# cgtuebingen/3D-RE-GEN

Measured on AMD Instinct MI355X. Metric: objects/sec (50-step Hunyuan3D-2 DiT + 256^3 marching cubes), higher is better.
Workload: dtype bf16; 1 GPU; configs[1]: 5 synthetic 512x512 RGBA crops per GPU, Hunyuan3D-2 full dims bf16, 50 flow-matching steps x CFG 2, 257^3 grid query + Lewiner marching cubes; weights=seeded synthetic, objects_total=5, objects_per_launch=4, parallelism=object-parallel x1

## Files before the change

### 3d-re-gen_amd/csrc/attn.hip

```cpp
#include <hip/hip_runtime.h>
#include <cstdio>
#include <stddef.h>
#include <stdint.h>

#include <type_traits>

#include "kernels.h"
#include "prof.h"

namespace r3g {
namespace {

typedef __attribute__((ext_vector_type(8))) __bf16 bf16x8;
typedef __attribute__((ext_vector_type(4))) __bf16 bf16x4;
typedef __attribute__((ext_vector_type(16))) float f32x16;
typedef __attribute__((ext_vector_type(8))) float f32x8;

constexpr int KV_TILE = 64;
constexpr int TILE_B = KV_TILE * 64 * 2;
constexpr int STAGE_B = 2 * TILE_B;

typedef __attribute__((ext_vector_type(2))) __bf16 bf16x2;
typedef __attribute__((ext_vector_type(2))) float f32x2;

__device__ __forceinline__ uint32_t pack_bf16(float a, float b) {
    const f32x2 v = {a, b};
    const bf16x2 h = __builtin_convertvector(v, bf16x2);
    return *reinterpret_cast<const uint32_t*>(&h);
}
// ... 42 lines not shown
                                                            offsetof(AttnEntry, lq));
}
__device__ __forceinline__ AttnEntry attn_entry(const AttnArgs& p, int e) {
    AttnEntry r{};
    if (!p.ragged) {
        r.lq = p.Lq; r.lk = p.Lk; r.bias_key = -1; r.buf = e;
        return r;
    }
    typedef const char __attribute__((address_space(4)))* kernarg_ptr;
    kernarg_ptr ka = (kernarg_ptr)__builtin_amdgcn_kernarg_segment_ptr();
    const AttnEntry __attribute__((address_space(4)))* t =
        (const AttnEntry __attribute__((address_space(4)))*)(ka + offsetof(AttnArgs, ent) + (size_t)e * sizeof(AttnEntry));
    r.lq = t->lq; r.lk = t->lk; r.bias_key = t->bias_key; r.bias_log2 = t->bias_log2; r.buf = t->buf;
    return r;
}
__device__ __forceinline__ int64_t attn_entry_out_row(int e, int q) {
    typedef const char __attribute__((address_space(4)))* kernarg_ptr;
    kernarg_ptr ka = (kernarg_ptr)__builtin_amdgcn_kernarg_segment_ptr();
    const AttnEntry __attribute__((address_space(4)))* t =
        (const AttnEntry __attribute__((address_space(4)))*)(ka + offsetof(AttnArgs, ent) + (size_t)e * sizeof(AttnEntry));
    const int split = t->o_split;
    return q < split ? t->o_row0 + q : t->o_row_split + (q - split);
}
template <int QT>
__device__ __forceinline__ void attn_work_item(const AttnArgs& p, int item, int& eb, int& hd, int& qt) {
    if (p.ragged) {
        int per_head = 0;
        for (int e = 0; e < p.B; ++e) per_head += (attn_entry_lq(p, e) + QT - 1) / QT;
        hd = item / per_head;
        int rem = item - hd * per_head;
        eb = 0;
        for (;;) {
            const int n = (attn_entry_lq(p, eb) + QT - 1) / QT;
            if (rem < n || eb + 1 >= p.B) break;
            rem -= n;
            ++eb;
        }
        qt = rem;
    } else {
        const int ntq0 = (p.Lq + QT - 1) / QT;
        const int per_head = ntq0 * p.B;
        hd = item / per_head;
        const int rem = item - hd * per_head;
        eb = rem / ntq0;
        qt = rem - eb * ntq0;
    }
}

template <bool GLDS, int ABL = 0>
__global__ __launch_bounds__(256, 2) void attn_kernel(AttnArgs p) {
    __shared__ __attribute__((aligned(16))) char smem[2 * STAGE_B];
    const int tid = threadIdx.x, lane = tid & 63;
    const int wid = __builtin_amdgcn_readfirstlane(tid >> 6);
    const int hd = blockIdx.y;
    const int eb = blockIdx.z;
    const AttnEntry en = attn_entry(p, eb);
    const int b = en.buf;
    const int ql = lane & 31, hh = lane >> 5;
    const int q = blockIdx.x * 128 + wid * 32 + ql;
    const int Lq = en.lq, Lk = en.lk;
    if ((int)blockIdx.x * 128 >= Lq) return;
    const int kvb = p.kv_batch_stride_zero ? 0 : b;
// ... 391 lines not shown
__device__ __forceinline__ float sum16(const float (&pe)[16]) {
    typedef __attribute__((ext_vector_type(2))) float f2;
    f2 ps = (f2){pe[0], pe[1]};
#pragma unroll
    for (int r = 2; r < 16; r += 2) ps += (f2){pe[r], pe[r + 1]};
    return ps[0] + ps[1];
}
constexpr float SCORE_LIMIT = 8.f;

__device__ __forceinline__ f32x16 mfma_32x32x16_fresh(const bf16x8& a, const bf16x8& b, const f32x16& c) {
    f32x16 d;
    asm volatile("s_nop 1\n\tv_mfma_f32_32x32x16_bf16 %0, %1, %2, %3" : "=&v"(d) : "v"(a), "v"(b), "v"(c));
    return d;
}

template <bool GLDS, bool PIPE, int NW, int ABL = 0, int VAR = 0>
__global__ __launch_bounds__(NW * 64, (PIPE || NW == 8) ? 2 : 3) void attn2_kernel(AttnArgs p) {
    __shared__ __attribute__((aligned(16))) char smem[(PIPE ? 3 : 2) * STAGE_B];
    const int tid = threadIdx.x, lane = tid & 63;
    const int wid = __builtin_amdgcn_readfirstlane(tid >> 6);
    const int ql = lane & 31, hh = lane >> 5;
    int eb, hd, qt;
    {
        const int nwg = gridDim.x, orig = blockIdx.x;
        const int qn = nwg >> 3, rn = nwg & 7, xcd = orig & 7;
        const int item = (xcd < rn ? xcd * (qn + 1) : rn * (qn + 1) + (xcd - rn) * qn) + (orig >> 3);
        constexpr int QT = NW * 32;
        attn_work_item<QT>(p, item, eb, hd, qt);
    }
    const AttnEntry en = attn_entry(p, eb);
    const int b = en.buf;
    const int q = qt * (NW * 32) + wid * 32 + ql;
    const int Lq = en.lq, Lk = en.lk;
    const int kvb = p.kv_batch_stride_zero ? 0 : b;
    const uint16_t* Qg = p.Q + (((int64_t)b * p.H + hd) * p.Lq_pad) * 64;
    const uint16_t* Kg = p.K + (((int64_t)kvb * p.H + hd) * p.Lk_pad) * 64;
    const uint16_t* Vtg = p.Vt + (((int64_t)kvb * p.H + hd) * 64) * (int64_t)p.Lk_pad;

    bf16x8 qf[4];
    {
        const int qrow = q < p.Lq_pad ? q : p.Lq_pad - 1;
#pragma unroll
        for (int ks = 0; ks < 4; ++ks)
            qf[ks] = *reinterpret_cast<const bf16x8*>(Qg + (int64_t)qrow * 64 + ks * 16 + hh * 8);
    }
    if (!p.q_prescaled) {
        const float sc = p.scale * 1.4426950408889634f;
#pragma unroll
        for (int ks = 0; ks < 4; ++ks) {
            union { bf16x8 v; uint32_t u[4]; } w;
            w.v = qf[ks];
// ... 32 lines not shown
    auto stage = [&](int t, char* dst) {
        if constexpr (GLDS) {
            const char* kt = reinterpret_cast<const char*>(Kg + (int64_t)t * (KV_TILE * 64));
            const char* vt = reinterpret_cast<const char*>(Vtg + (int64_t)t * KV_TILE);
#pragma unroll
            for (int i = 0; i < PPW; ++i) {
                if constexpr ((VAR & 4) != 0) {
                    lds_dma16_unseen(kt, koff[i], smem_lds + (uint32_t)(dst - smem) + (wid * PPW + i) * 1024);
                    lds_dma16_unseen(vt, voff[i], smem_lds + (uint32_t)(dst - smem) + TILE_B + (wid * PPW + i) * 1024);
                    continue;
                }
                __builtin_amdgcn_global_load_lds((const __attribute__((address_space(1))) void*)(kt + (size_t)koff[i]),
                                                 (__attribute__((address_space(3))) void*)(dst + (wid * PPW + i) * 1024), 16, 0, 0);
                __builtin_amdgcn_global_load_lds((const __attribute__((address_space(1))) void*)(vt + (size_t)voff[i]),
                                                 (__attribute__((address_space(3))) void*)(dst + TILE_B + (wid * PPW + i) * 1024),
                                                 16, 0, 0);
            }
        } else {
            static_assert(GLDS || NW == 4, "register staging is only built for 4-wave workgroups");
            stage_kv<false>(Kg, Vtg, p.Lk_pad, t * KV_TILE, dst, wid, lane, tid);
        }
    };
    const bool pad_tail = ntiles * KV_TILE > Lk;
    if constexpr (PIPE) {
        auto qk = [&](const char* buf, int kb, bool from_zero) {
            f32x16 sc_;
            const bf16x8 k0 = *reinterpret_cast<const bf16x8*>(buf + off[kb]);
            if (from_zero) {
                f32x16 z;
#pragma unroll
                for (int r = 0; r < 16; ++r) z[r] = 0.f;
                sc_ = __builtin_amdgcn_mfma_f32_32x32x16_bf16(k0, qf[0], z, 0, 0, 0);
            } else {
                sc_ = mfma_32x32x16_fresh(k0, qf[0], negm);
            }
#pragma unroll
            for (int ks = 1; ks < 4; ++ks) {
                const bf16x8 kf = *reinterpret_cast<const bf16x8*>(buf + (off[kb] ^ (ks << 5)));
                sc_ = __builtin_amdgcn_mfma_f32_32x32x16_bf16(kf, qf[ks], sc_, 0, 0, 0);
            }
            return sc_;
        };
        auto mask_block = [&](f32x16& sc_, int t, int kb) {
            const int key_base = t * KV_TILE + kb * 32 + 4 * hh;
#pragma unroll
            for (int r = 0; r < 16; ++r) {
// ... 72 lines not shown
                if (t > 0) mask_block(sA, t, 0);
                mask_block(sB, t, 1);
            }
            softmax_block(sA, &sB, pk);
            pv(cur, 0, pk);
            if constexpr (decltype(has_next)::value) {
                sA = qk(nxt, 0, false);
                softmax_block(sB, &sA, pk);
            } else {
                softmax_block(sB, nullptr, pk);
            }
            pv(cur, 1, pk);
            asm volatile("s_waitcnt vmcnt(0)" ::: "memory");
            __syncthreads();
        };
        int slot = 0;
        for (int t = 0; t < ntiles - 1; ++t) {
            tile(std::false_type{}, std::true_type{}, t, slot);
            slot = slot == 2 ? 0 : slot + 1;
        }
        if (pad_tail) tile(std::true_type{}, std::false_type{}, ntiles - 1, slot);
        else tile(std::false_type{}, std::false_type{}, ntiles - 1, slot);
    } else {
    unsigned long long sticky = 0;
    const unsigned long long valid_lanes = __ballot(q < Lq);
    auto pass = [&](auto FAST) __attribute__((always_inline)) {
    constexpr bool kFast = decltype(FAST)::value;
#pragma unroll
    for (int r = 0; r < 16; ++r) { o[0][r] = 0.f; o[1][r] = 0.f; negm[r] = 0.f; }
    m_run = 0.f;
    l_run = 0.f;
    stage(0, smem);
    asm volatile("s_waitcnt vmcnt(0)" ::: "memory");
    __syncthreads();

    auto tile = [&](auto masked, auto first, const int t) {
        const char* cur = smem + (t & 1) * STAGE_B;
        if constexpr ((VAR & 4) != 0) __builtin_amdgcn_s_waitcnt(0x0F70);
        if (!(ABL & 16) && t + 1 < ntiles) stage(t + 1, smem + ((t + 1) & 1) * STAGE_B);
#pragma unroll
        for (int kb = 0; kb < 2; ++kb) {
            constexpr bool kFirst = decltype(first)::value;
            const bool first_block = kFirst && kb == 0;
            f32x16 s;
            if constexpr ((ABL & 8) != 0) {
                const float tv = __int_as_float(0x3f800000 + (t << 8));
#pragma unroll
                for (int r = 0; r < 16; ++r) s[r] = negm[r] + tv * (float)(r + 1) * 1e-3f;
                if (!(ABL & 128)) {
#pragma unroll
                    for (int ks = 0; ks < 4; ++ks) {
                        const bf16x8 kf = *reinterpret_cast<const bf16x8*>(cur + (off[kb] ^ (ks << 5)));
                        asm volatile("" ::"v"(kf));
                    }
                }
            } else {
                const bf16x8 k0 = (ABL & 128) ? qf[1] : *reinterpret_cast<const bf16x8*>(cur + off[kb]);
                if (first_block) {
                    f32x16 z;
#pragma unroll
                    for (int r = 0; r < 16; ++r) z[r] = 0.f;
                    s = __builtin_amdgcn_mfma_f32_32x32x16_bf16(k0, qf[0], z, 0, 0, 0);
                } else {
                    s = mfma_32x32x16_fresh(k0, qf[0], negm);
                }
#pragma unroll
// ... 113 lines not shown
        pk[J - 1] = pack_bf16(st.ea, st.eb);
        asm volatile("" : "+v"(pk[J - 1]));
    }
    st.ea = a;
    st.eb = b;
    if (J == 7) {
        pk[7] = pack_bf16(a, b);
        st.ps0 += a;
        st.ps1 += b;
        asm volatile("" : "+v"(pk[7]));
    }
    asm volatile("" : "+v"(st.ps0), "+v"(st.ps1), "+v"(st.ea), "+v"(st.eb));
}

template <int NW, int VAR = 0>
__global__ __launch_bounds__(NW * 64, 2) void attn3_kernel(AttnArgs p) {
    __shared__ __attribute__((aligned(16))) char smem[2 * STAGE_B];
    const int tid = threadIdx.x, lane = tid & 63;
    const int wid = __builtin_amdgcn_readfirstlane(tid >> 6);
    const int ql = lane & 31, hh = lane >> 5;
    constexpr int QT = NW * 64;
    int eb, hd, qt;
    {
        const int nwg = gridDim.x, orig = blockIdx.x;
        const int qn = nwg >> 3, rn = nwg & 7, xcd = orig & 7;
        const int item = (xcd < rn ? xcd * (qn + 1) : rn * (qn + 1) + (xcd - rn) * qn) + (orig >> 3);
        attn_work_item<QT>(p, item, eb, hd, qt);
    }
    const AttnEntry en = attn_entry(p, eb);
    const int b = en.buf;
    const int q0 = qt * QT + wid * 64 + ql;
    const int Lq = en.lq, Lk = en.lk;
    const int kvb = p.kv_batch_stride_zero ? 0 : b;
    const uint16_t* Qg = p.Q + (((int64_t)b * p.H + hd) * p.Lq_pad) * 64;
    const uint16_t* Kg = p.K + (((int64_t)kvb * p.H + hd) * p.Lk_pad) * 64;
    const uint16_t* Vtg = p.Vt + (((int64_t)kvb * p.H + hd) * 64) * (int64_t)p.Lk_pad;

    bf16x8 qf[2][4];
#pragma unroll
    for (int qb = 0; qb < 2; ++qb) {
        const int q = q0 + qb * 32;
        const int qrow = q < p.Lq_pad ? q : p.Lq_pad - 1;
#pragma unroll
        for (int ks = 0; ks < 4; ++ks)
            qf[qb][ks] = *reinterpret_cast<const bf16x8*>(Qg + (int64_t)qrow * 64 + ks * 16 + hh * 8);
    }
    if (!p.q_prescaled) {
        const float sc = p.scale * 1.4426950408889634f;
#pragma unroll
        for (int qb = 0; qb < 2; ++qb)
// ... 251 lines not shown
                odd.y = pack_bf16(o[qb][db][8 * gp + 6] * inv, o[qb][db][8 * gp + 7] * inv);
                const u32x2 rx = __builtin_amdgcn_permlane32_swap(even.x, odd.x, false, false);
                const u32x2 ry = __builtin_amdgcn_permlane32_swap(even.y, odd.y, false, false);
                uint4 out;
                out.x = rx[0]; out.y = ry[0]; out.z = rx[1]; out.w = ry[1];
                if (q < Lq) *reinterpret_cast<uint4*>(dst + db * 32 + 16 * gp + 8 * hh) = out;
            }
    }
}


template <bool STAMP, int PRIO>
__global__ __launch_bounds__(768, 3) void attn6_kernel(AttnArgs p, unsigned long long* __restrict__ stamps) {
    extern __shared__ __attribute__((aligned(16))) char smem6[];
    char* const smem = smem6;
    constexpr int R = 4;
    const int tid = threadIdx.x, lane = tid & 63;
    const int wid = __builtin_amdgcn_readfirstlane(tid >> 6);
    const int grp = wid >> 2;
    const int ql = lane & 31, hh = lane >> 5;
    constexpr int QT = 384;
    int eb, hd, qt;
    {
        const int nwg = gridDim.x, orig = blockIdx.x;
        const int qn = nwg >> 3, rn = nwg & 7, xcd = orig & 7;
        const int item = (xcd < rn ? xcd * (qn + 1) : rn * (qn + 1) + (xcd - rn) * qn) + (orig >> 3);
        attn_work_item<QT>(p, item, eb, hd, qt);
    }
    const AttnEntry en = attn_entry(p, eb);
    const int b = en.buf;
    const int q = qt * QT + wid * 32 + ql;
    const int Lq = en.lq, Lk = en.lk;
    const int kvb = p.kv_batch_stride_zero ? 0 : b;
    const uint16_t* Qg = p.Q + (((int64_t)b * p.H + hd) * p.Lq_pad) * 64;
    const uint16_t* Kg = p.K + (((int64_t)kvb * p.H + hd) * p.Lk_pad) * 64;
    const uint16_t* Vtg = p.Vt + (((int64_t)kvb * p.H + hd) * 64) * (int64_t)p.Lk_pad;

    const int ntiles = (Lk + KV_TILE - 1) / KV_TILE;
    const int nblk = 2 * ntiles;
    const bool stager = wid < 8;
    int koff, voff;
    {
        const int row = (wid & 7) * 8 + (lane >> 3);
        const int kc = (lane & 7) ^ ((row >> 1) & 7);
        koff = row * 64 + kc * 8;
        voff = row * p.Lk_pad + kc * 8;
    }
    auto stage = [&](int t) {
        char* dst = smem + (t % R) * STAGE_B;
        const uint16_t* kt = Kg + (int64_t)t * (KV_TILE * 64);
// ... 184 lines not shown
                uint4 out;
                out.x = rx[0]; out.y = ry[0]; out.z = rx[1]; out.w = ry[1];
                if (q < Lq) *reinterpret_cast<uint4*>(dst + db * 32 + 16 * gp + 8 * hh) = out;
            }
    }
    for (int g = grp; g < 2; ++g) R3G_PHASE_END();
#undef R3G_PHASE_END
}

}

static bool g_attn_glds = true;
static bool g_attn_pipelined = false;
static int g_attn_ablate = 0;
void attn_set_ablate(int mask) { g_attn_ablate = mask; }
void attn_set_glds(bool on) { g_attn_glds = on; }
void attn_set_pipelined(bool on) { g_attn_pipelined = on; }

static int g_attn_gen = 7;
static int g_attn_variant = 1;
void attn_set_variant(int v) { if (v >= 0 && v <= 1) g_attn_variant = v; }
static int g_attn_interleave = 0;
void attn_set_interleave(int v) { g_attn_interleave = v != 0; }
static int g_attn_async_stage = 1;
void attn_set_async_stage(int v) { g_attn_async_stage = v != 0; }
static int g_wide6_min_items = 2048;
void attn_set_wide_min(int items) { if (items > 0) g_wide6_min_items = items; }
void attn_set_generation(int gen) { if ((gen >= 1 && gen <= 7) || gen == 9) g_attn_gen = gen; }
static int g_attn6_prio = 1;
void attn_set_prio(int v) { if (v >= 0 && v <= 2) g_attn6_prio = v; }
static int g_attn_stamps = 0;
void attn_set_stamps(int on) { g_attn_stamps = on; }

float attn_q_scale(float scale) { return (g_attn_gen >= 2 && !g_attn_pipelined) ? scale * 1.4426950408889634f : 1.0f; }

hipError_t attention_launch(const AttnArgs& p, hipStream_t s) {
    if (p.ragged) {
        if (p.B < 1 || p.B > kAttnMaxEntries) return hipErrorInvalidValue;
        for (int b = 0; b < p.B; ++b) {
            const AttnEntry& en = p.ent[b];
            if (en.lq <= 0 || en.lk <= 0 || en.lq > p.Lq_pad || en.lk > p.Lk_pad || en.buf < 0) return hipErrorInvalidValue;
            const int nt = (en.lk + 63) / 64;
            if (en.bias_key >= 0 && (en.bias_key < (nt - 1) * 64 || nt * 64 == en.lk || en.bias_key >= en.lk))
                return hipErrorInvalidValue;
        }
    }
    if (p.Lq_pad % 128 || p.Lk_pad % 64 || p.Lk <= 0 || p.Lq <= 0 || p.Lk > p.Lk_pad || p.Lq > p.Lq_pad)
        return hipErrorInvalidValue;
    double pairs = (double)p.B * p.Lq * p.Lk;
    if (p.ragged) {
        pairs = 0;
        for (int b = 0; b < p.B; ++b) pairs += (double)p.ent[b].lq * p.ent[b].lk;
    }
    ProfScope ps(PC_ATTN, 4.0 * p.H * pairs * 64, s);
    if (g_attn_gen >= 2 && !g_attn_pipelined) {
        auto count = [&](int qtile) {
            int n = 0;
            if (p.ragged) for (int b = 0; b < p.B; ++b) n += (p.ent[b].lq + qtile - 1) / qtile;
            else n = ((p.Lq + qtile - 1) / qtile) * p.B;
// ... 93 lines not shown
```

### 3d-re-gen_amd/csrc/kernels.h

```cpp
#ifndef R3G_KERNELS_H
#define R3G_KERNELS_H
#include <hip/hip_runtime.h>
#include <stdint.h>

namespace r3g {

enum GemmEpilogue {
    EPI_BF16 = 0,
    EPI_BF16_GELU_TANH = 1,
    EPI_BF16_GELU_ERF = 2,
    EPI_RESID_F32 = 3,
    EPI_F32 = 4,
    EPI_QKV = 5,
    EPI_RESID_BF16 = 6,
    EPI_FP8_GELU_ERF = 7,
    EPI_RESID_F16 = 8,
    EPI_RESID_BF16_LND = 9,
    EPI_RESID_BF16_ST = 10,
    EPI_BF16_GELU_ERF_LNF = 11,
};

enum QkNorm { QKN_NONE = 0, QKN_RMS = 1, QKN_LAYERNORM = 2 };

enum QkvLayout {
// ... 88 lines not shown
void gemm_set_wide_epilogue(bool on);

constexpr int kAttnMaxEntries = 8;
struct AttnEntry {
    int lq, lk;
    int o_split, bias_key;
    int64_t o_row0, o_row_split;
    float bias_log2;
    int buf;
};
struct AttnArgs {
    const uint16_t* Q;
    const uint16_t* K;
    const uint16_t* Vt;
    uint16_t* O;
    int64_t ldo, strideO;
    int B, H;
    int Lq, Lq_pad;
    int Lk, Lk_pad;
    int kv_batch_stride_zero;
    float scale;
    int q_prescaled;
    int ragged;
    AttnEntry ent[kAttnMaxEntries];
};

hipError_t attention_launch(const AttnArgs& p, hipStream_t s);
float attn_q_scale(float scale);
void attn_set_wide_min(int items);
void attn_set_prio(int v);
void attn_set_stamps(int on);
void attn_set_generation(int gen);
void ln_set_rows4_min(int rows);
void ln_set_modes(bool on);
void ln_set_rows_per_wave(int rows);
void ln_set_fixed_count(bool on);

struct LnArgs {
    const float* x; int64_t ldx;
    int x_bf16;
    uint16_t* y; int64_t ldy;
    uint8_t* y8; int64_t ldy8; float* y_scale;
    int64_t x_batch_stride, y_batch_stride;
    const float* w; const float* b;
    const float* scale; const float* shift; int64_t mod_stride;
    int seg2_row0, seg2_row1;
    const float* scale2; const float* shift2;
    int rows, C, rows_per_batch;
    float eps;
};
hipError_t layernorm_launch(const LnArgs& p, hipStream_t s);
// ... 67 lines not shown
```

### 3d-re-gen_amd/csrc/model.cpp

```cpp
#include <hip/hip_runtime.h>

#include <algorithm>
#include <cmath>
#include <cstdarg>
#include <cstdio>
#include <cstring>
#include <string>
#include <unordered_map>
#include <vector>

#include "../../include/r3g.h"
#include "kernels.h"
#include "mesh_kernels.h"
#include "prof.h"
#include "r3g_ctx.h"

namespace r3g {

struct Tensor {
    const void* p;
    int dtype;
    int64_t rows, cols;
};

// ... 4 lines not shown
    int64_t ldw = 0;
};

static inline int64_t rup(int64_t v, int64_t m) { return (v + m - 1) / m * m; }

static bool g_overlap_mlp = false;
static bool g_group_streams = true;
static bool g_fuse_qkv = true;
static bool g_batch_mods = true;
static int g_geo_fp8 = 0;
constexpr float kGeoHiddenScale = 1.0f / 16.0f;
static bool g_geo_resid_bf16 = true;
static bool g_cfg_dedup = true;
static unsigned g_option_epoch = 0;
static long long g_geo_q_cache_bytes = -1;
static bool g_geo_q_cache = true;
static bool g_dit_f16_guard = true;
static bool g_geo_ln3_fold = true;
static bool g_geo_lnd_fused = true;
static int64_t g_geo_q_cache_builds = 0;
static int64_t g_dit_groups = 0;
static int g_dit_f16_fallbacks = 0;
static bool g_dit_resid_f16 = true;
static bool g_skip_zero_step = true;
static int g_flow_first_step = 0, g_flow_last_step = 1 << 30;

struct Model {
    r3g_model_config c{};
    std::unordered_map<std::string, Tensor> w;
    std::unordered_map<std::string, float> scalars;
    int T = 0, Tpad = 0, Lc = 0, Lcpad = 0, H = 0, Hd = 0, W = 0, Wh = 0, Hc = 0, Hch = 0, Fc = 0;
    int cin_pad = 0, qc = 0;
    char* arena = nullptr;
    size_t arena_bytes = 0;
    float* f32a = nullptr;
    uint16_t* xn = nullptr;
    uint16_t* qkv = nullptr;
    uint16_t *Q = nullptr, *K = nullptr, *Vt = nullptr;
    uint16_t* cat = nullptr;
    uint16_t* hid = nullptr;
    uint16_t* inb = nullptr;
    float* small = nullptr;
    float *temb = nullptr, *th = nullptr, *vec = nullptr, *mods = nullptr, *v2 = nullptr;
    float* z = nullptr;
    uint16_t *geoK = nullptr, *geoVt = nullptr;
    bool have_z = false;
// ... 463 lines not shown
        R3G_RC(get_lin(m, bi + "_attn.proj", true, &li));
        R3G_RC(get_lin(m, bt + "_attn.proj", true, &lt));
        R3G_RC(gemm_pair(gemm_args(d.cat, catld, 0, li, 0, H, d.f32a, H, 0, TX0, H, epi_res, mi + 2 * H, 0), 1,
                         gemm_args(catt, catld, 0, lt, 0, H, xt, H, 0, Mtxt, H, epi_res, mt + 2 * H, 0), 1, s));
        R3G_RC(ln_streams(mi + 4 * H, mi + 3 * H, mt + 4 * H, mt + 3 * H));
        R3G_RC(get_lin(m, bi + "_mlp.0", true, &li));
        R3G_RC(get_lin(m, bt + "_mlp.0", true, &lt));
        R3G_RC(gemm_pair(gemm_args(d.xn, H, 0, li, 0, mh, d.cat + H, catld, 0, TX0, H, EPI_BF16_GELU_TANH, nullptr, 0), 1,
                         gemm_args(xnt, H, 0, lt, 0, mh, catt + H, catld, 0, Mtxt, H, EPI_BF16_GELU_TANH, nullptr, 0), 1, s));
        R3G_RC(get_lin(m, bi + "_mlp.2", true, &li));
        R3G_RC(get_lin(m, bt + "_mlp.2", true, &lt));
        R3G_RC(gemm_pair(gemm_args(d.cat + H, catld, 0, li, 0, H, d.f32a, H, 0, TX0, mh, epi_res, mi + 5 * H, 0), 1,
                         gemm_args(catt + H, catld, 0, lt, 0, H, xt, H, 0, Mtxt, mh, epi_res, mt + 5 * H, 0), 1, s));
    }
    const bool overlap = g_overlap_mlp && c.dit_depth_single > 0;
    if (overlap && !m.aux) {
        R3G_TRY(hipStreamCreateWithFlags(&m.aux, hipStreamNonBlocking));
        R3G_TRY(hipEventCreateWithFlags(&m.ev_fork, hipEventDisableTiming));
        R3G_TRY(hipEventCreateWithFlags(&m.ev_join, hipEventDisableTiming));
    }
    for (int i = 0; i < c.dit_depth_single; ++i) {
        const std::string blk = fmt("model.single_blocks.%d", i);
        const float* mm = m.mod_all + m.mod_off[2 * c.dit_depth_double + i];
        R3G_RC(layernorm(d.f32a, H, 0, d.xn, H, 0, Rall, 1, H, nullptr, nullptr, mm + H, mm, 0, 1e-6f, s, xfmt));
        R3G_RC(get_lin(m, blk + ".linear1", true, &l));
        QkvSplitArgs q;
        R3G_RC(qkv_args(blk + ".norm.query_norm.scale", blk + ".norm.key_norm.scale", &q));
        const GemmArgs pq = qkv_gemm_args(d.xn, 0, l, Rall, q, 4 * NB, d.seg_all, &d.h_seg_all);
        auto launch_qkv = [&]() -> int {
            hipError_t e = gemm_launch(pq, 1, s);
            if (e != hipSuccess) return hip_fail(e, "gemm_launch(qkv dedup)");
            return R3G_OK;
        };
        hipStream_t sm = s;
        if (overlap) {
            R3G_RC(launch_qkv());
            R3G_TRY(hipEventRecord(m.ev_fork, s));
            R3G_TRY(hipStreamWaitEvent(m.aux, m.ev_fork, 0));
            sm = m.aux;
        }
        if (overlap) {
            R3G_RC(gemm(d.xn, H, 0, l, 3 * H, mh, d.cat + H, catld, 0, Rall, H, EPI_BF16_GELU_TANH, nullptr, 0, 1, sm));
            R3G_TRY(hipEventRecord(m.ev_join, m.aux));
        } else {
            const GemmArgs pm = gemm_args(d.xn, H, 0, l, 3 * H, mh, d.cat + H, catld, 0, Rall, H, EPI_BF16_GELU_TANH, nullptr, 0);
            hipError_t e1 = gemm_launch_qkv_mlp(pq, pm, s);
            if (e1 != hipSuccess) return hip_fail(e1, "gemm_launch_qkv_mlp");
        }
        hipError_t e = attention_launch(at, s);
        if (e != hipSuccess) return hip_fail(e, "attention_launch(dedup)");
        if (overlap) R3G_TRY(hipStreamWaitEvent(s, m.ev_join, 0));
        R3G_RC(get_lin(m, blk + ".linear2", true, &l));
        R3G_RC(gemm(d.cat, catld, 0, l, 0, H, d.f32a, H, 0, Rall, H + mh, epi_res, mm + 2 * H, 0, 1, s));
    }
    const float* fm = m.mod_all + m.mod_off[2 * c.dit_depth_double + c.dit_depth_single];
    R3G_RC(layernorm(d.f32a, H, 0, d.xn, H, 0, TX0, 1, H, nullptr, nullptr, fm + H, fm, 0, 1e-6f, s, xfmt));
    R3G_RC(get_lin(m, "model.final_layer.linear", true, &l));
    R3G_RC(gemm(d.xn, H, 0, l, 0, c.dit_in_channels, out2, c.dit_in_channels, 0, TX0, H, EPI_F32, nullptr, 0, 1, s));
    return R3G_OK;
}

static int vae_decode(Model& m, const float* latents, hipStream_t s) {
    const r3g_model_config& c = m.c;
    const int W = m.W, Nl = c.vae_num_latents, heads = m.Wh;
    Lin l;
    R3G_TRY(cast_pad_launch(latents, c.vae_embed_dim, m.inb, m.cin_pad, Nl, c.vae_embed_dim, m.cin_pad,
                            1.0f / c.vae_scale_factor, s));
    R3G_RC(get_lin(m, "vae.post_kl", true, &l));
    R3G_RC(gemm(m.inb, m.cin_pad, 0, l, 0, W, m.z, W, 0, Nl, m.cin_pad, EPI_F32, nullptr, 0, 1, s));
    const float *lw, *lb;
    for (int i = 0; i < c.vae_layers; ++i) {
        const std::string blk = fmt("vae.transformer.resblocks.%d", i);
        R3G_RC(get_vec(m, blk + ".ln_1.weight", W, &lw));
        R3G_RC(get_vec(m, blk + ".ln_1.bias", W, &lb));
        R3G_RC(layernorm(m.z, W, 0, m.xn, W, 0, Nl, 1, W, lw, lb, nullptr, nullptr, 0, 1e-6f, s));
        R3G_RC(get_lin(m, blk + ".attn.c_qkv", c.vae_qkv_bias != 0, &l));
// ... 693 lines not shown
    if (!d_a8 || !d_w8 || !d_scale_a || !d_scale_w || !d_c) return fail(R3G_ERR_INVALID, "r3g_op_gemm_fp8: null argument");
    GemmArgs p{};
    p.A = reinterpret_cast<const uint16_t*>(d_a8); p.lda = lda; p.W = reinterpret_cast<const uint16_t*>(d_w8); p.ldw = ldw;
    p.bias = d_bias; p.C = d_c; p.ldc = ldc; p.gate = d_gate;
    p.M = m_; p.N = n_; p.K = k_; p.epi = epilogue;
    hipError_t e = gemm_fp8_launch(p, d_scale_a, d_scale_w, (hipStream_t)stream);
    if (e != hipSuccess) return hip_fail(e, "r3g_op_gemm_fp8 (needs K % 256 == 0, 16-byte aligned rows, N % 4 == 0, a bf16 / residual epilogue)");
    return R3G_OK;
}

int r3g_op_attention(const uint16_t* d_q, const uint16_t* d_k, const uint16_t* d_vt, uint16_t* d_o, int batch, int heads,
                     int lq, int lq_pad, int lk, int lk_pad, int shared_kv, int use_lds_dma, void* stream) {
    AttnArgs p{};
    p.Q = d_q; p.K = d_k; p.Vt = d_vt; p.O = d_o; p.ldo = (int64_t)heads * 64; p.strideO = (int64_t)lq * heads * 64;
    p.B = batch; p.H = heads; p.Lq = lq; p.Lq_pad = lq_pad; p.Lk = lk; p.Lk_pad = lk_pad;
    p.kv_batch_stride_zero = shared_kv; p.scale = 0.125f;
    attn_set_glds(use_lds_dma != 0);
    hipError_t e = attention_launch(p, (hipStream_t)stream);
    attn_set_glds(true);
    if (e != hipSuccess) return hip_fail(e, "r3g_op_attention");
    return R3G_OK;
}

int r3g_prof_enable(int on) {
    prof_enable(on != 0);
    return R3G_OK;
}

int r3g_prof_read(int64_t* counts, double* ms, double* work, int n) {
    if (!counts || !ms || !work || n < PC_COUNT) return fail(R3G_ERR_INVALID, "r3g_prof_read: need %d slots", (int)PC_COUNT);
    long long c[PC_COUNT];
    prof_read(c, ms, work);
    for (int i = 0; i < PC_COUNT; ++i) counts[i] = c[i];
    return R3G_OK;
}

int r3g_prof_read_bytes(double* bytes, int n) {
    if (!bytes || n < PC_COUNT) return fail(R3G_ERR_INVALID, "r3g_prof_read_bytes: need %d slots", (int)PC_COUNT);
    prof_read_bytes(bytes);
    return R3G_OK;
}

int r3g_set_option(const char* name, int value) {
    if (!name) return fail(R3G_ERR_INVALID, "r3g_set_option: null name");
    ++g_option_epoch;
    if (!strcmp(name, "fuse_qkv")) g_fuse_qkv = value != 0;
// ... 7 lines not shown
    else if (!strcmp(name, "dit_f16_guard")) g_dit_f16_guard = value != 0;
    else if (!strcmp(name, "gelu_pk")) gemm_set_gelu_pk(value != 0);
    else if (!strcmp(name, "geo_fp8")) g_geo_fp8 = value >= 0 && value <= 3 ? value : 0;
    else if (!strcmp(name, "group_streams")) g_group_streams = value != 0;
    else if (!strcmp(name, "overlap_mlp")) g_overlap_mlp = value != 0;
    else if (!strcmp(name, "gemm_waves")) gemm_set_config(value);
    else if (!strcmp(name, "gemm_raster")) gemm_set_raster(value);
    else if (!strcmp(name, "gemm_auto_rule")) gemm_set_auto_rule(value, 0);
    else if (!strcmp(name, "gemm_num_cu")) gemm_set_auto_rule(-1, value);
    else if (!strcmp(name, "gemm_wide_epilogue")) gemm_set_wide_epilogue(value != 0);
    else if (!strcmp(name, "gemm_phased")) gemm_set_phased(value != 0);
    else if (!strcmp(name, "gemm_persistent")) gemm_set_persistent(value != 0);
    else if (!strcmp(name, "gemm_persistent_resid")) gemm_set_persistent_resid(value);
    else if (!strcmp(name, "gemm_splitk")) gemm_set_splitk(value != 0);
    else if (!strcmp(name, "gemm_splitk128")) gemm_set_splitk128(value != 0);
    else if (!strcmp(name, "conv_implicit")) gemm_set_conv_implicit(value != 0);
    else if (!strcmp(name, "gemm_xcd_walk")) gemm_set_xcd_walk(value != 0);
    else if (!strcmp(name, "ln_modes")) ln_set_modes(value != 0);
    else if (!strcmp(name, "geo_lnd_fused")) g_geo_lnd_fused = value != 0;
    else if (!strcmp(name, "geo_ln3_fold")) g_geo_ln3_fold = value != 0;
    else if (!strcmp(name, "attn_variant")) attn_set_variant(value);
    else if (!strcmp(name, "attn_interleave")) attn_set_interleave(value);
    else if (!strcmp(name, "attn_async_stage")) attn_set_async_stage(value);
    else if (!strcmp(name, "gemm_epi_slices")) gemm_set_epi_slices(value != 0);
    else if (!strcmp(name, "gemm_mixed")) gemm_set_mixed(value != 0);
    else if (!strcmp(name, "gemm_persistent_qkv")) gemm_set_persistent_qkv(value != 0);
    else if (!strcmp(name, "flow_first_step")) g_flow_first_step = value;
    else if (!strcmp(name, "flow_last_step")) g_flow_last_step = value < 0 ? (1 << 30) : value;
    else if (!strcmp(name, "attn_pipelined")) attn_set_pipelined(value != 0);
    else if (!strcmp(name, "attn_ablate")) attn_set_ablate(value);
    else if (!strcmp(name, "attn_generation")) attn_set_generation(value);
    else if (!strcmp(name, "attn_stamps")) attn_set_stamps(value);
    else if (!strcmp(name, "attn_prio")) attn_set_prio(value);
    else if (!strcmp(name, "attn_wide_min")) attn_set_wide_min(value);
    else if (!strcmp(name, "ln_rows")) ln_set_rows_per_wave(value);
    else if (!strcmp(name, "ln_rows4_min")) ln_set_rows4_min(value);
    else if (!strcmp(name, "ln_fixed")) ln_set_fixed_count(value != 0);
    else if (!strcmp(name, "floater_by_vertex")) mesh_set_floater_by_vertex(value != 0);
    else if (!strcmp(name, "mc_rows")) mc_set_rows_per_wave(value);
    else if (!strcmp(name, "mc_deferred")) mc_set_deferred(value != 0);
    else if (!strcmp(name, "lds_dma")) { gemm_set_glds(value != 0); attn_set_glds(value != 0); }
    else return fail(R3G_ERR_INVALID, "r3g_set_option: unknown option '%s'", name);
    return R3G_OK;
}

int r3g_set_staging(int use_lds_dma) {
// ... 7 lines not shown
```

### 3d-re-gen_amd/r3g/ffi.py

```python
import ctypes
import os

_PKG = os.path.dirname(os.path.dirname(os.path.abspath(__file__)))
LIB_PATH = os.environ.get("R3G_LIBRARY") or os.path.join(_PKG, "libr3g.so")

R3G_ERR_LEVEL_RANGE = -10
R3G_ERR_NO_SURFACE = -11


class R3GError(RuntimeError):
    def __init__(self, code, msg):
        super().__init__("libr3g error %d: %s" % (code, msg))
        self.code = code


class LevelRangeError(ValueError):
    """skimage: ValueError('Surface level must be within volume data range.')"""


class NoSurfaceError(RuntimeError):
    """skimage: RuntimeError('No surface found at the given iso value.')"""


_P = ctypes.c_void_p
# ... 36 lines not shown
    "r3g_grid_query_hier": (_I, [_P, _D, _I, _D, _D, _I, _P, _I64P, _I, _P]),
    "r3g_unet_create": (_I, [_P, _P]),
    "r3g_unet_set_tensor": (_I, [_P, ctypes.c_char_p, _P, _I, ctypes.c_int64, ctypes.c_int64]),
    "r3g_unet_resnet": (_I, [_P, ctypes.c_char_p, _P, _I, _I, _I, _I, _P, _P, _P]),
    "r3g_unet_transformer": (_I, [_P, ctypes.c_char_p, _P, _I, _I, _I, _P, _I, _P]),
    "r3g_unet_downsample": (_I, [_P, ctypes.c_char_p, _P, _I, _I, _I, _P, _P]),
    "r3g_unet_down_block": (_I, [_P, ctypes.c_char_p, _P, _I, _I, _I, _I, _P, _P, _I, _I, _I, _P, _P, _P]),
    "r3g_unet_forward": (_I, [_P, _P, _I, _I, ctypes.c_float, _P, _I, _P, _P]),
    "r3g_unet_mid_block": (_I, [_P, ctypes.c_char_p, _P, _I, _I, _I, _P, _P, _I, _P, _P]),
    "r3g_unet_forward_mv": (_I, [_P, _P, _I, _I, ctypes.c_float, _P, _I, _I, _P, _I, ctypes.c_float, ctypes.c_float, _P, _P]),
    "r3g_unet_transformer_mv": (_I, [_P, ctypes.c_char_p, _P, _I, _I, _I, _P, _I, _I, _I, ctypes.c_float, ctypes.c_float, _P]),
    "r3g_unet_condition": (_I, [_P, ctypes.c_char_p, _P, _P, _P]),
    "r3g_aekl_decode": (_I, [_P, _P, _I, _I, _P, _P]),
    "r3g_aekl_encode": (_I, [_P, _P, _I, _I, _P, _P]),
    "r3g_sched_pix2pix_input": (_I, [_P, _P, _I, ctypes.c_int64, ctypes.c_float, _P, _P]),
    "r3g_sched_model_input": (_I, [_P, _I, _P, _I, ctypes.c_int64, ctypes.c_float, _P, _P]),
    "r3g_sched_cfg_combine": (_I, [_P, _P, ctypes.c_int64, ctypes.c_float, _P, _P]),
    "r3g_sched_euler_ancestral_step": (_I, [_P, _P, _P, ctypes.c_int64, ctypes.c_float, ctypes.c_float, _I, _P]),
    "r3g_op_gemm": (_I, [_P, ctypes.c_int64, _P, ctypes.c_int64, _P, _P, ctypes.c_int64, _P, _I, _I, _I, _I, _I, _P]),
    "r3g_op_gemm_splitk": (_I, [_P, ctypes.c_int64, _P, ctypes.c_int64, _P, _P, ctypes.c_int64, _P, _I, _I, _I, _I, _P, ctypes.c_int64, _P, _P]),
    "r3g_op_quant_fp8": (_I, [_P, ctypes.c_int64, _I, _I, _P, ctypes.c_int64, _P, _P]),
    "r3g_op_gemm_fp8": (_I, [_P, ctypes.c_int64, _P, _P, ctypes.c_int64, _P, _P, _P, ctypes.c_int64, _P, _I, _I, _I, _I, _P]),
    "r3g_op_attention": (_I, [_P, _P, _P, _P, _I, _I, _I, _I, _I, _I, _I, _I, _P]),
    "r3g_set_staging": (_I, [_I]),
    "r3g_set_option": (_I, [ctypes.c_char_p, _I]),
    "r3g_get_counter": (_I, [ctypes.c_char_p, _P]),
    "r3g_prof_enable": (_I, [_I]),
    "r3g_prof_read": (_I, [_P, _P, _P, _I]),
    "r3g_prof_read_bytes": (_I, [_P, _I]),
}


class ModelConfig(ctypes.Structure):
    _fields_ = [(n, ctypes.c_int32) for n in (
        "dit_in_channels", "dit_context_dim", "dit_hidden", "dit_heads", "dit_depth_double", "dit_depth_single",
        "dit_mlp_hidden", "dit_qkv_bias")] + [("dit_time_factor", ctypes.c_float)] + [(n, ctypes.c_int32) for n in (
            "vae_num_latents", "vae_embed_dim", "vae_width", "vae_heads", "vae_layers", "vae_num_freqs",
            "vae_include_pi", "vae_qkv_bias", "vae_qk_norm", "vae_mlp_ratio", "vae_ln_post")] + [
        ("vae_scale_factor", ctypes.c_float)] + [(n, ctypes.c_int32) for n in (
            "cond_image_size", "cond_patch", "cond_hidden", "cond_layers", "cond_heads", "cond_ffn_hidden")] + [
        ("cond_ln_eps", ctypes.c_float), ("grid_chunk", ctypes.c_int32)]

class UnetConfig(ctypes.Structure):
    _fields_ = [(n, ctypes.c_int32) for n in ("max_hw", "max_channels", "temb_dim", "ctx_dim", "ctx_tokens", "groups")] + [
        ("resnet_eps", ctypes.c_float)] + [(n, ctypes.c_int32) for n in ("n_levels", "layers_per_block", "in_channels", "out_channels")] + [
        ("block_out_channels", ctypes.c_int32 * 4)]
# ... 68 lines not shown
```

### include/r3g.h

```cpp
#ifndef R3G_H
#define R3G_H

#include <stddef.h>
#include <stdint.h>

#ifdef __cplusplus
extern "C" {
#endif

#define R3G_VERSION 100

#define R3G_OK 0
#define R3G_ERR_INVALID (-1)
#define R3G_ERR_HIP (-2)
#define R3G_ERR_NO_DEVICE (-3)
#define R3G_ERR_STATE (-4)
#define R3G_ERR_LEVEL_RANGE (-10)
#define R3G_ERR_NO_SURFACE (-11)

typedef struct r3g_ctx r3g_ctx;

int r3g_version(void);
const char* r3g_last_error(void);

// ... 106 lines not shown
                            int tokens, int n_views, int flags, float mva_scale, float ref_scale, void* stream);
int r3g_unet_condition(r3g_ctx* ctx, const char* prefix, const void** d_ptr, int64_t* rows, int64_t* cols);
int r3g_unet_mid_block(r3g_ctx* ctx, const char* prefix, const float* d_x, int height, int width, int channels,
                       const float* d_temb, const uint16_t* d_ctx, int tokens, float* d_out, void* stream);

int r3g_aekl_decode(r3g_ctx* ctx, const float* d_latent, int height, int width, float* d_image, void* stream);
int r3g_aekl_encode(r3g_ctx* ctx, const float* d_image, int height, int width, float* d_moments, void* stream);

int r3g_sched_model_input(const float* d_latent, int channels, const float* d_cond, int cond_channels, int64_t pixels, float sigma,
                          float* d_out, void* stream);
int r3g_sched_pix2pix_input(const float* d_latent, const float* d_image_latent, int channels, int64_t pixels, float sigma,
                            float* d_out, void* stream);
int r3g_sched_cfg_combine(const float* d_uncond, const float* d_cond, int64_t n, float guidance_scale, float* d_out, void* stream);
int r3g_sched_euler_ancestral_step(float* d_sample, const float* d_model_out, const float* d_noise, int64_t n, float sigma_from,
                                   float sigma_to, int prediction_type, void* stream);

int r3g_op_gemm(const uint16_t* d_a, int64_t lda, const uint16_t* d_w, int64_t ldw, const float* d_bias, void* d_c,
                int64_t ldc, const float* d_gate, int m, int n, int k, int epilogue, int use_lds_dma, void* stream);
int r3g_op_gemm_splitk(const uint16_t* d_a, int64_t lda, const uint16_t* d_w, int64_t ldw, const float* d_bias, float* d_c, int64_t ldc,
                       const float* d_gate, int m, int n, int k, int epilogue, float* d_ws, int64_t ws_elems, int* slices,
                       void* stream);
int r3g_op_attention(const uint16_t* d_q, const uint16_t* d_k, const uint16_t* d_vt, uint16_t* d_o, int batch, int heads,
                     int lq, int lq_pad, int lk, int lk_pad, int shared_kv, int use_lds_dma, void* stream);
int r3g_op_quant_fp8(const uint16_t* d_x, int64_t ldx, int rows, int k, uint8_t* d_q, int64_t ldq, float* d_scale, void* stream);
int r3g_op_gemm_fp8(const uint8_t* d_a8, int64_t lda, const float* d_scale_a, const uint8_t* d_w8, int64_t ldw,
                    const float* d_scale_w, const float* d_bias, void* d_c, int64_t ldc, const float* d_gate, int m, int n,
                    int k, int epilogue, void* stream);
int r3g_prof_enable(int on);
int r3g_prof_read(int64_t* counts, double* ms, double* work, int n);
int r3g_prof_read_bytes(double* bytes, int n);
int r3g_set_option(const char* name, int value);
int r3g_get_counter(const char* name, int64_t* value);
int r3g_set_staging(int use_lds_dma);

#ifdef __cplusplus
}
#endif
#endif
```

Before: 0.8148 objects/sec.

## Skip padded attention work and compute only latent rows in last DiT block

```diff
diff --git a/3d-re-gen_amd/csrc/attn.hip b/3d-re-gen_amd/csrc/attn.hip
--- a/3d-re-gen_amd/csrc/attn.hip
+++ b/3d-re-gen_amd/csrc/attn.hip
@@ -5,6 +5,7 @@
 
 #include <type_traits>
 
+#include "attn_work.h"
 #include "kernels.h"
 #include "prof.h"
 
@@ -93,22 +94,22 @@
     const int split = t->o_split;
     return q < split ? t->o_row0 + q : t->o_row_split + (q - split);
 }
+__device__ __forceinline__ int attn_entry_lk(const AttnArgs& p, int e) {
+    typedef const char __attribute__((address_space(4)))* kernarg_ptr;
+    kernarg_ptr ka = (kernarg_ptr)__builtin_amdgcn_kernarg_segment_ptr();
+    return *(const int __attribute__((address_space(4)))*)(ka + offsetof(AttnArgs, ent) + (size_t)e * sizeof(AttnEntry) +
+                                                            offsetof(AttnEntry, lk));
+}
 template <int QT>
-__device__ __forceinline__ void attn_work_item(const AttnArgs& p, int item, int& eb, int& hd, int& qt) {
+__device__ __forceinline__ void attn_work_item(const AttnArgs& p, int& eb, int& hd, int& qt) {
+    const int nwg = gridDim.x, orig = blockIdx.x;
     if (p.ragged) {
-        int per_head = 0;
-        for (int e = 0; e < p.B; ++e) per_head += (attn_entry_lq(p, e) + QT - 1) / QT;
-        hd = item / per_head;
-        int rem = item - hd * per_head;
-        eb = 0;
-        for (;;) {
-            const int n = (attn_entry_lq(p, eb) + QT - 1) / QT;
-            if (rem < n || eb + 1 >= p.B) break;
-            rem -= n;
-            ++eb;
-        }
-        qt = rem;
+        attn_work_decode(p.item_order, nwg, orig, p.B, [&](int e) { return (attn_entry_lq(p, e) + QT - 1) / QT; },
+                         [&](int e) { return (attn_entry_lk(p, e) + kAttnKeyTile - 1) / kAttnKeyTile; }, eb, hd, qt);
     } else {
+        int start, count;
+        attn_xcd_range(nwg, orig & 7, start, count);
+        const int item = start + (orig >> 3);
         const int ntq0 = (p.Lq + QT - 1) / QT;
         const int per_head = ntq0 * p.B;
         hd = item / per_head;
@@ -546,11 +547,8 @@
     const int ql = lane & 31, hh = lane >> 5;
     int eb, hd, qt;
     {
-        const int nwg = gridDim.x, orig = blockIdx.x;
-        const int qn = nwg >> 3, rn = nwg & 7, xcd = orig & 7;
-        const int item = (xcd < rn ? xcd * (qn + 1) : rn * (qn + 1) + (xcd - rn) * qn) + (orig >> 3);
         constexpr int QT = NW * 32;
-        attn_work_item<QT>(p, item, eb, hd, qt);
+        attn_work_item<QT>(p, eb, hd, qt);
     }
     const AttnEntry en = attn_entry(p, eb);
     const int b = en.buf;
@@ -629,6 +627,8 @@
         }
     };
     const bool pad_tail = ntiles * KV_TILE > Lk;
+    const bool wave_idle = !PIPE && ABL == 0 && p.skip_padded && qt * (NW * 32) + wid * 32 >= Lq;
+    const bool tail_block_empty = p.skip_padded && Lk - (ntiles - 1) * KV_TILE <= 32;
     if constexpr (PIPE) {
         auto qk = [&](const char* buf, int kb, bool from_zero) {
             f32x16 sc_;
@@ -747,6 +747,24 @@
         if (pad_tail) tile(std::true_type{}, std::false_type{}, ntiles - 1, slot);
         else tile(std::false_type{}, std::false_type{}, ntiles - 1, slot);
     } else {
+    if (wave_idle) {
+        auto idle_pass = [&]() __attribute__((always_inline)) {
+            stage(0, smem);
+            asm volatile("s_waitcnt vmcnt(0)" ::: "memory");
+            __syncthreads();
+            for (int t = 0; t < ntiles; ++t) {
+                if constexpr ((VAR & 4) != 0) __builtin_amdgcn_s_waitcnt(0x0F70);
+                if (t + 1 < ntiles) stage(t + 1, smem + ((t + 1) & 1) * STAGE_B);
+                asm volatile("s_waitcnt vmcnt(0)" ::: "memory");
+                __syncthreads();
+            }
+        };
+        idle_pass();
+        if constexpr ((VAR & 1) != 0 && ABL == 0) {
+            if (__syncthreads_or(0)) idle_pass();
+        }
+        return;
+    }
     unsigned long long sticky = 0;
     const unsigned long long valid_lanes = __ballot(q < Lq);
     auto pass = [&](auto FAST) __attribute__((always_inline)) {
@@ -767,6 +785,9 @@
         for (int kb = 0; kb < 2; ++kb) {
             constexpr bool kFirst = decltype(first)::value;
             const bool first_block = kFirst && kb == 0;
+            if constexpr (decltype(masked)::value) {
+                if (kb == 1 && tail_block_empty) continue;
+            }
             f32x16 s;
             if constexpr ((ABL & 8) != 0) {
                 const float tv = __int_as_float(0x3f800000 + (t << 8));
@@ -926,10 +947,7 @@
     constexpr int QT = NW * 64;
     int eb, hd, qt;
     {
-        const int nwg = gridDim.x, orig = blockIdx.x;
-        const int qn = nwg >> 3, rn = nwg & 7, xcd = orig & 7;
-        const int item = (xcd < rn ? xcd * (qn + 1) : rn * (qn + 1) + (xcd - rn) * qn) + (orig >> 3);
-        attn_work_item<QT>(p, item, eb, hd, qt);
+        attn_work_item<QT>(p, eb, hd, qt);
     }
     const AttnEntry en = attn_entry(p, eb);
     const int b = en.buf;
@@ -1227,10 +1245,7 @@
     constexpr int QT = 384;
     int eb, hd, qt;
     {
-        const int nwg = gridDim.x, orig = blockIdx.x;
-        const int qn = nwg >> 3, rn = nwg & 7, xcd = orig & 7;
-        const int item = (xcd < rn ? xcd * (qn + 1) : rn * (qn + 1) + (xcd - rn) * qn) + (orig >> 3);
-        attn_work_item<QT>(p, item, eb, hd, qt);
+        attn_work_item<QT>(p, eb, hd, qt);
     }
     const AttnEntry en = attn_entry(p, eb);
     const int b = en.buf;
@@ -1461,6 +1476,10 @@
 void attn_set_variant(int v) { if (v >= 0 && v <= 1) g_attn_variant = v; }
 static int g_attn_interleave = 0;
 void attn_set_interleave(int v) { g_attn_interleave = v != 0; }
+static int g_attn_skip_padded = 1;
+void attn_set_skip_padded(int v) { g_attn_skip_padded = v != 0; }
+static int g_attn_item_order = kAttnOrderBase;
+void attn_set_item_order(int v) { if (v >= 0 && v < kAttnOrders) g_attn_item_order = v; }
 static int g_attn_async_stage = 1;
 void attn_set_async_stage(int v) { g_attn_async_stage = v != 0; }
 static int g_wide6_min_items = 2048;
@@ -1473,7 +1492,10 @@
 
 float attn_q_scale(float scale) { return (g_attn_gen >= 2 && !g_attn_pipelined) ? scale * 1.4426950408889634f : 1.0f; }
 
-hipError_t attention_launch(const AttnArgs& p, hipStream_t s) {
+hipError_t attention_launch(const AttnArgs& args, hipStream_t s) {
+    AttnArgs p = args;
+    p.skip_padded = g_attn_skip_padded;
+    p.item_order = p.ragged ? g_attn_item_order : kAttnOrderBase;
     if (p.ragged) {
         if (p.B < 1 || p.B > kAttnMaxEntries) return hipErrorInvalidValue;
         for (int b = 0; b < p.B; ++b) {
diff --git a/3d-re-gen_amd/csrc/attn_work.h b/3d-re-gen_amd/csrc/attn_work.h
--- /dev/null
+++ b/3d-re-gen_amd/csrc/attn_work.h
@@ -0,0 +1,90 @@
+#ifndef R3G_ATTN_WORK_H
+#define R3G_ATTN_WORK_H
+
+#if defined(__HIPCC__)
+#define R3G_AW __host__ __device__ __forceinline__
+#else
+#define R3G_AW static inline
+#endif
+
+namespace r3g {
+
+constexpr int kAttnOrderBase = 0;
+constexpr int kAttnOrderLongFirst = 1;
+constexpr int kAttnOrders = 2;
+constexpr int kAttnKeyTile = 64;
+
+R3G_AW void attn_xcd_range(int nwg, int xcd, int& start, int& count) {
+    const int qn = nwg >> 3, rn = nwg & 7;
+    start = xcd < rn ? xcd * (qn + 1) : rn * (qn + 1) + (xcd - rn) * qn;
+    count = qn + (xcd < rn ? 1 : 0);
+}
+
+template <class NQ>
+R3G_AW void attn_item_base(int item, int B, NQ nq, int& eb, int& hd, int& qt) {
+    int per_head = 0;
+    for (int e = 0; e < B; ++e) per_head += nq(e);
+    hd = item / per_head;
+    int rem = item - hd * per_head;
+    eb = 0;
+    for (;;) {
+        const int n = nq(eb);
+        if (rem < n || eb + 1 >= B) break;
+        rem -= n;
+        ++eb;
+    }
+    qt = rem;
+}
+
+template <class NQ, class NK>
+R3G_AW void attn_work_decode(int order, int nwg, int orig, int B, NQ nq, NK nk, int& eb, int& hd, int& qt) {
+    int start, count;
+    attn_xcd_range(nwg, orig & 7, start, count);
+    int j = orig >> 3;
+    if (order != kAttnOrderLongFirst) {
+        attn_item_base(start + j, B, nq, eb, hd, qt);
+        return;
+    }
+    int per_head = 0;
+    for (int e = 0; e < B; ++e) per_head += nq(e);
+    int bound = 0x7fffffff;
+    for (;;) {
+        int v = -1;
+        for (int e = 0; e < B; ++e) {
+            const int k = nk(e);
+            if (k < bound && k > v) v = k;
+        }
+        if (v < 0) break;
+        int in_head = 0;
+        for (int e = 0; e < B; ++e)
+            if (nk(e) == v) in_head += nq(e);
+        auto before = [&](int x) {
+            const int h = x / per_head, r = x - h * per_head;
+            int g = 0, off = 0;
+            for (int e = 0; e < B; ++e) {
+                const int n = nq(e);
+                if (nk(e) == v) g += r - off <= 0 ? 0 : (r - off < n ? r - off : n);
+                off += n;
+            }
+            return h * in_head + g;
+        };
+        const int f0 = before(start), c = before(start + count) - f0;
+        if (j < c) {
+            const int k = f0 + j;
+            hd = k / in_head;
+            int rem = k - hd * in_head;
+            for (int e = 0; e < B; ++e) {
+                if (nk(e) != v) continue;
+                const int n = nq(e);
+                if (rem < n) { eb = e; qt = rem; return; }
+                rem -= n;
+            }
+        }
+        j -= c;
+        bound = v;
+    }
+    attn_item_base(start + (orig >> 3), B, nq, eb, hd, qt);
+}
+
+}
+#endif
diff --git a/3d-re-gen_amd/csrc/kernels.h b/3d-re-gen_amd/csrc/kernels.h
--- a/3d-re-gen_amd/csrc/kernels.h
+++ b/3d-re-gen_amd/csrc/kernels.h
@@ -134,11 +134,14 @@
     float scale;
     int q_prescaled;
     int ragged;
+    int skip_padded, item_order;
     AttnEntry ent[kAttnMaxEntries];
 };
 
 hipError_t attention_launch(const AttnArgs& p, hipStream_t s);
 float attn_q_scale(float scale);
+void attn_set_skip_padded(int v);
+void attn_set_item_order(int v);
 void attn_set_wide_min(int items);
 void attn_set_prio(int v);
 void attn_set_stamps(int on);
diff --git a/3d-re-gen_amd/csrc/model.cpp b/3d-re-gen_amd/csrc/model.cpp
--- a/3d-re-gen_amd/csrc/model.cpp
+++ b/3d-re-gen_amd/csrc/model.cpp
@@ -50,6 +50,7 @@
 static int64_t g_dit_groups = 0;
 static int g_dit_f16_fallbacks = 0;
 static bool g_dit_resid_f16 = true;
+static bool g_dit_last_block_latents_only = true;
 static bool g_skip_zero_step = true;
 static int g_flow_first_step = 0, g_flow_last_step = 1 << 30;
 
@@ -559,6 +560,11 @@
     for (int i = 0; i < c.dit_depth_single; ++i) {
         const std::string blk = fmt("model.single_blocks.%d", i);
         const float* mm = m.mod_all + m.mod_off[2 * c.dit_depth_double + i];
+        const bool lat_only = g_dit_last_block_latents_only && i == c.dit_depth_single - 1;
+        const int Mout = lat_only ? TX0 : Rall;
+        AttnArgs at_blk = at;
+        if (lat_only)
+            for (int e = 0; e < 2 * NB; ++e) at_blk.ent[e].lq = Nl;
         R3G_RC(layernorm(d.f32a, H, 0, d.xn, H, 0, Rall, 1, H, nullptr, nullptr, mm + H, mm, 0, 1e-6f, s, xfmt));
         R3G_RC(get_lin(m, blk + ".linear1", true, &l));
         QkvSplitArgs q;
@@ -577,18 +583,18 @@
             sm = m.aux;
         }
         if (overlap) {
-            R3G_RC(gemm(d.xn, H, 0, l, 3 * H, mh, d.cat + H, catld, 0, Rall, H, EPI_BF16_GELU_TANH, nullptr, 0, 1, sm));
+            R3G_RC(gemm(d.xn, H, 0, l, 3 * H, mh, d.cat + H, catld, 0, Mout, H, EPI_BF16_GELU_TANH, nullptr, 0, 1, sm));
             R3G_TRY(hipEventRecord(m.ev_join, m.aux));
         } else {
-            const GemmArgs pm = gemm_args(d.xn, H, 0, l, 3 * H, mh, d.cat + H, catld, 0, Rall, H, EPI_BF16_GELU_TANH, nullptr, 0);
+            const GemmArgs pm = gemm_args(d.xn, H, 0, l, 3 * H, mh, d.cat + H, catld, 0, Mout, H, EPI_BF16_GELU_TANH, nullptr, 0);
             hipError_t e1 = gemm_launch_qkv_mlp(pq, pm, s);
             if (e1 != hipSuccess) return hip_fail(e1, "gemm_launch_qkv_mlp");
         }
-        hipError_t e = attention_launch(at, s);
+        hipError_t e = attention_launch(at_blk, s);
         if (e != hipSuccess) return hip_fail(e, "attention_launch(dedup)");
         if (overlap) R3G_TRY(hipStreamWaitEvent(s, m.ev_join, 0));
         R3G_RC(get_lin(m, blk + ".linear2", true, &l));
-        R3G_RC(gemm(d.cat, catld, 0, l, 0, H, d.f32a, H, 0, Rall, H + mh, epi_res, mm + 2 * H, 0, 1, s));
+        R3G_RC(gemm(d.cat, catld, 0, l, 0, H, d.f32a, H, 0, Mout, H + mh, epi_res, mm + 2 * H, 0, 1, s));
     }
     const float* fm = m.mod_all + m.mod_off[2 * c.dit_depth_double + c.dit_depth_single];
     R3G_RC(layernorm(d.f32a, H, 0, d.xn, H, 0, TX0, 1, H, nullptr, nullptr, fm + H, fm, 0, 1e-6f, s, xfmt));
@@ -1328,6 +1334,29 @@
     return R3G_OK;
 }
 
+int r3g_op_attention_ragged(const uint16_t* d_q, const uint16_t* d_k, const uint16_t* d_vt, uint16_t* d_o, int heads, int lq_pad,
+                            int lk_pad, int64_t ldo, int n_entries, const int* lq, const int* lk, const int* buf,
+                            const int64_t* o_row0, const int* o_split, const int64_t* o_row_split, const int* bias_key,
+                            const float* bias_log2, void* stream) {
+    if (!d_q || !d_k || !d_vt || !d_o || !lq || !lk || !buf || !o_row0 || !o_split || !o_row_split || !bias_key || !bias_log2)
+        return fail(R3G_ERR_INVALID, "r3g_op_attention_ragged: null argument");
+    if (n_entries < 1 || n_entries > kAttnMaxEntries)
+        return fail(R3G_ERR_INVALID, "r3g_op_attention_ragged: 1 .. %d entries", kAttnMaxEntries);
+    AttnArgs p{};
+    p.Q = d_q; p.K = d_k; p.Vt = d_vt; p.O = d_o; p.ldo = ldo; p.strideO = 0;
+    p.B = n_entries; p.H = heads; p.Lq_pad = lq_pad; p.Lk_pad = lk_pad; p.scale = 0.125f;
+    p.ragged = 1;
+    for (int e = 0; e < n_entries; ++e) {
+        AttnEntry& en = p.ent[e];
+        en.lq = lq[e]; en.lk = lk[e]; en.buf = buf[e]; en.o_row0 = o_row0[e]; en.o_split = o_split[e];
+        en.o_row_split = o_row_split[e]; en.bias_key = bias_key[e]; en.bias_log2 = bias_log2[e];
+        p.Lq = std::max(p.Lq, en.lq); p.Lk = std::max(p.Lk, en.lk);
+    }
+    hipError_t e = attention_launch(p, (hipStream_t)stream);
+    if (e != hipSuccess) return hip_fail(e, "r3g_op_attention_ragged (entry lengths within the padded ones, a weighted key inside a padded last key tile)");
+    return R3G_OK;
+}
+
 int r3g_prof_enable(int on) {
     prof_enable(on != 0);
     return R3G_OK;
@@ -1381,6 +1410,9 @@
     else if (!strcmp(name, "attn_variant")) attn_set_variant(value);
     else if (!strcmp(name, "attn_interleave")) attn_set_interleave(value);
     else if (!strcmp(name, "attn_async_stage")) attn_set_async_stage(value);
+    else if (!strcmp(name, "dit_last_block_latents_only")) g_dit_last_block_latents_only = value != 0;
+    else if (!strcmp(name, "attn_skip_padded")) attn_set_skip_padded(value);
+    else if (!strcmp(name, "attn_item_order")) attn_set_item_order(value);
     else if (!strcmp(name, "gemm_epi_slices")) gemm_set_epi_slices(value != 0);
     else if (!strcmp(name, "gemm_mixed")) gemm_set_mixed(value != 0);
     else if (!strcmp(name, "gemm_persistent_qkv")) gemm_set_persistent_qkv(value != 0);
diff --git a/3d-re-gen_amd/r3g/ffi.py b/3d-re-gen_amd/r3g/ffi.py
--- a/3d-re-gen_amd/r3g/ffi.py
+++ b/3d-re-gen_amd/r3g/ffi.py
@@ -82,6 +82,7 @@
     "r3g_op_quant_fp8": (_I, [_P, ctypes.c_int64, _I, _I, _P, ctypes.c_int64, _P, _P]),
     "r3g_op_gemm_fp8": (_I, [_P, ctypes.c_int64, _P, _P, ctypes.c_int64, _P, _P, _P, ctypes.c_int64, _P, _I, _I, _I, _I, _P]),
     "r3g_op_attention": (_I, [_P, _P, _P, _P, _I, _I, _I, _I, _I, _I, _I, _I, _P]),
+    "r3g_op_attention_ragged": (_I, [_P, _P, _P, _P, _I, _I, _I, ctypes.c_int64, _I, _P, _P, _P, _P, _P, _P, _P, _P, _P]),
     "r3g_set_staging": (_I, [_I]),
     "r3g_set_option": (_I, [ctypes.c_char_p, _I]),
     "r3g_get_counter": (_I, [ctypes.c_char_p, _P]),
diff --git a/include/r3g.h b/include/r3g.h
--- a/include/r3g.h
+++ b/include/r3g.h
@@ -152,6 +152,10 @@
                        void* stream);
 int r3g_op_attention(const uint16_t* d_q, const uint16_t* d_k, const uint16_t* d_vt, uint16_t* d_o, int batch, int heads,
                      int lq, int lq_pad, int lk, int lk_pad, int shared_kv, int use_lds_dma, void* stream);
+int r3g_op_attention_ragged(const uint16_t* d_q, const uint16_t* d_k, const uint16_t* d_vt, uint16_t* d_o, int heads, int lq_pad,
+                            int lk_pad, int64_t ldo, int n_entries, const int* lq, const int* lk, const int* buf,
+                            const int64_t* o_row0, const int* o_split, const int64_t* o_row_split, const int* bias_key,
+                            const float* bias_log2, void* stream);
 int r3g_op_quant_fp8(const uint16_t* d_x, int64_t ldx, int rows, int k, uint8_t* d_q, int64_t ldq, float* d_scale, void* stream);
 int r3g_op_gemm_fp8(const uint8_t* d_a8, int64_t lda, const float* d_scale_a, const uint8_t* d_w8, int64_t ldw,
                     const float* d_scale_w, const float* d_bias, void* d_c, int64_t ldc, const float* d_gate, int m, int n,
```

New measurement: 0.8193 objects/sec, median of 6. About the same (+0.6%).
